# hulop/SfM

Hardware: AMD Instinct MI355X
Metric: BA iterations/sec + residual-evals/sec (cams x pts x obs); 1/2/4/8 GPU (higher is better)
Workload: dtype f64; 1 GPU; C3 per GPU: full BA solve (LM + DENSE_SCHUR, Ceres default options); cams=500, points=200000, observations=2000000, points_per_gpu=200000, obs_per_gpu=2000000, views_per_point=10, parallelism=single GPU, reduced_camera_factor=single GPU

## Files before the change

include/sfm_amd.h:

```cpp
#ifndef SFM_AMD_H_
#define SFM_AMD_H_

#include <stdint.h>

#ifdef __cplusplus
extern "C" {
#endif

#define SFM_ABI_VERSION 1

#define SFM_OK 0
#define SFM_EINVAL (-22)
#define SFM_ENOMEM (-12)
#define SFM_ENODEV (-19)
#define SFM_EIO (-5)
#define SFM_ENOTSUP (-95)

#define SFM_BA_STRUCT_ONLY 0
#define SFM_BA_POSE_ONLY 1
#define SFM_BA_STRUCT_AND_POSE 2

typedef struct sfm_ba_options {
  int32_t max_num_iterations;
  int32_t max_num_consecutive_invalid_steps;
// ... 36 lines not shown
  int32_t step_is_valid;
  int32_t step_is_successful;
  int32_t reserved;
  double cost;
  double cost_change;
  double gradient_max_norm;
  double step_norm;
  double relative_decrease;
  double trust_region_radius;
} sfm_ba_iteration;

typedef struct sfm_ba_handle sfm_ba_handle;

int32_t sfm_abi_version(void);
const char* sfm_last_error(void);
void sfm_ba_default_options(sfm_ba_options* opts);
int32_t sfm_device_count(void);

int sfm_ba_solve(const sfm_ba_options* opts, int32_t mode, int64_t n_obs, const double* obs_uv,
                 const int32_t* cam_idx, const int32_t* pt_idx, int32_t n_cams, const double* K9, double* rot,
                 double* t, int32_t n_pts, double* X, sfm_ba_summary* summary, sfm_ba_iteration* trace,
                 int32_t trace_cap, int32_t* trace_len);

int sfm_ba_create(int32_t device, sfm_ba_handle** out);
int sfm_ba_destroy(sfm_ba_handle* h);
int sfm_ba_set_problem(sfm_ba_handle* h, int64_t n_obs, const double* obs_uv, const int32_t* cam_idx,
                       const int32_t* pt_idx, int32_t n_cams, const double* K9, const double* rot, const double* t,
                       int32_t n_pts, const double* X);
int sfm_ba_reset_parameters(sfm_ba_handle* h);
int sfm_ba_solve_resident(sfm_ba_handle* h, const sfm_ba_options* opts, int32_t mode, sfm_ba_summary* summary,
                          sfm_ba_iteration* trace, int32_t trace_cap, int32_t* trace_len);
int sfm_ba_get_parameters(sfm_ba_handle* h, double* rot, double* t, double* X);
int sfm_ba_evaluate(sfm_ba_handle* h, double* cost, double* res, double* jac);
int sfm_ba_bench_jacobian(sfm_ba_handle* h, int32_t reps, double* avg_ms);
int sfm_ba_phase_times(sfm_ba_handle* h, double* ms9);
int sfm_ba_set_profiling(sfm_ba_handle* h, int32_t on);
int sfm_ba_sync(sfm_ba_handle* h);

int sfm_comm_unique_id(uint8_t out[128]);
int sfm_ba_set_comm(sfm_ba_handle* h, int32_t nranks, int32_t rank, const uint8_t id[128]);
typedef int (*sfm_allreduce_fn)(double* buf, int64_t count, int32_t op, void* user);
int sfm_ba_set_host_comm(sfm_ba_handle* h, int32_t nranks, int32_t rank, sfm_allreduce_fn fn, void* user);
#define SFM_COLL_ALLREDUCE 0
#define SFM_COLL_BROADCAST 1
#define SFM_COLL_REDUCE_SCATTER 2
#define SFM_COLL_REDUCE 3
typedef int (*sfm_collective_fn)(int32_t kind, double* buf, double* out, int64_t count, int32_t arg, void* user);
int sfm_ba_set_host_collectives(sfm_ba_handle* h, int32_t nranks, int32_t rank, sfm_collective_fn fn, void* user);
int sfm_ba_set_distributed_factor(sfm_ba_handle* h, int32_t panel_tiles);

int sfm_match_features(int32_t device, const double* pts0, const uint8_t* desc0, int32_t n0, const double* pts1,
                       const uint8_t* desc1, int32_t n1, int32_t desc_bytes, double ratio_test, double min_distance,
                       double max_distance, int32_t* idx0, int32_t* idx1, int32_t* n_matches);
int sfm_knn2_hamming(int32_t device, const uint8_t* desc0, int32_t n0, const uint8_t* desc1, int32_t n1,
                     int32_t desc_bytes, int32_t* best_idx, int32_t* best_dist, int32_t* second_idx,
                     int32_t* second_dist);

typedef struct sfm_matcher sfm_matcher;
int sfm_matcher_create(int32_t device, int32_t desc_bytes, sfm_matcher** out);
int sfm_matcher_destroy(sfm_matcher* h);
int sfm_matcher_push_frame(sfm_matcher* h, const double* pts, const double* pts_distorted, const uint8_t* desc,
                           int32_t n);
int sfm_matcher_match_subset(sfm_matcher* h, const int32_t* prev_idx, int32_t n_prev, const int32_t* curr_idx,
                             int32_t n_curr, double ratio_test, double min_distance, double max_distance,
                             int32_t* prev_match, int32_t* curr_match, int32_t* n_matches);
int sfm_matcher_store_keyframe(sfm_matcher* h, int32_t slot, const double* pts, const uint8_t* desc, int32_t n);
// ... 246 lines not shown
```

sfm_amd/_ffi.py:

```python
from __future__ import annotations

import ctypes
import os
from ctypes import POINTER, c_char_p, c_double, c_float, c_int, c_int32, c_int64, c_uint8, c_uint64, c_void_p

import numpy as np

_HERE = os.path.dirname(os.path.abspath(__file__))
LIB_PATH = os.environ.get("SFM_AMD_LIB") or os.path.join(_HERE, "libsfm_amd.so")


class SfmError(RuntimeError):

    def __init__(self, code: int, what: str, msg: str):
        super().__init__(f"{what} failed with {code}: {msg}")
        self.code = code


class BAOptions(ctypes.Structure):
    _fields_ = [
        ("max_num_iterations", c_int32),
        ("max_num_consecutive_invalid_steps", c_int32),
        ("jacobi_scaling", c_int32),
        ("reserved0", c_int32),
# ... 117 lines not shown


class GuidanceResult(ctypes.Structure):
    _fields_ = [
        ("centroid", c_double * 3),
        ("box_center", c_float * 2),
        ("box_size", c_float * 2),
        ("box_angle", c_float),
        ("n_points", c_int32),
        ("n_projected", c_int32),
        ("n_hull", c_int32),
        ("n_accepted", c_int32),
        ("area", c_double),
    ]


_SIGNATURES = {
    "sfm_abi_version": (c_int32, []),
    "sfm_last_error": (c_char_p, []),
    "sfm_ba_default_options": (None, [POINTER(BAOptions)]),
    "sfm_device_count": (c_int32, []),
    "sfm_ba_solve": (c_int, [POINTER(BAOptions), c_int32, c_int64, c_void_p, c_void_p, c_void_p, c_int32, c_void_p,
                             c_void_p, c_void_p, c_int32, c_void_p, POINTER(BASummary), c_void_p, c_int32,
                             POINTER(c_int32)]),
    "sfm_ba_create": (c_int, [c_int32, POINTER(c_void_p)]),
    "sfm_ba_destroy": (c_int, [c_void_p]),
    "sfm_ba_set_problem": (c_int, [c_void_p, c_int64, c_void_p, c_void_p, c_void_p, c_int32, c_void_p, c_void_p,
                                   c_void_p, c_int32, c_void_p]),
    "sfm_ba_reset_parameters": (c_int, [c_void_p]),
    "sfm_ba_solve_resident": (c_int, [c_void_p, POINTER(BAOptions), c_int32, POINTER(BASummary), c_void_p, c_int32,
                                      POINTER(c_int32)]),
    "sfm_ba_get_parameters": (c_int, [c_void_p, c_void_p, c_void_p, c_void_p]),
    "sfm_ba_evaluate": (c_int, [c_void_p, POINTER(c_double), c_void_p, c_void_p]),
    "sfm_ba_bench_jacobian": (c_int, [c_void_p, c_int32, POINTER(c_double)]),
    "sfm_ba_phase_times": (c_int, [c_void_p, c_void_p]),
    "sfm_ba_set_profiling": (c_int, [c_void_p, c_int32]),
    "sfm_ba_sync": (c_int, [c_void_p]),
    "sfm_comm_unique_id": (c_int, [c_void_p]),
    "sfm_ba_set_comm": (c_int, [c_void_p, c_int32, c_int32, c_void_p]),
    "sfm_ba_set_host_comm": (c_int, [c_void_p, c_int32, c_int32, c_void_p, c_void_p]),
    "sfm_ba_set_host_collectives": (c_int, [c_void_p, c_int32, c_int32, c_void_p, c_void_p]),
    "sfm_ba_set_distributed_factor": (c_int, [c_void_p, c_int32]),
    "sfm_match_features": (c_int, [c_int32, c_void_p, c_void_p, c_int32, c_void_p, c_void_p, c_int32, c_int32,
                                   c_double, c_double, c_double, c_void_p, c_void_p, POINTER(c_int32)]),
    "sfm_knn2_hamming": (c_int, [c_int32, c_void_p, c_int32, c_void_p, c_int32, c_int32, c_void_p, c_void_p,
                                 c_void_p, c_void_p]),
    "sfm_matcher_create": (c_int, [c_int32, c_int32, POINTER(c_void_p)]),
    "sfm_matcher_destroy": (c_int, [c_void_p]),
    "sfm_matcher_push_frame": (c_int, [c_void_p, c_void_p, c_void_p, c_void_p, c_int32]),
    "sfm_matcher_match_subset": (c_int, [c_void_p, c_void_p, c_int32, c_void_p, c_int32, c_double, c_double, c_double,
                                         c_void_p, c_void_p, POINTER(c_int32)]),
    "sfm_matcher_match_frames": (c_int, [c_void_p, c_int32, c_double, c_double, c_double, c_void_p, c_void_p,
                                         POINTER(c_int32)]),
    "sfm_matcher_match": (c_int, [c_void_p, c_void_p, c_void_p, c_int32, c_void_p, c_void_p, c_int32, c_double,
                                  c_double, c_double, c_void_p, c_void_p, POINTER(c_int32)]),
    "sfm_matcher_knn2": (c_int, [c_void_p, c_void_p, c_int32, c_void_p, c_int32, c_void_p, c_void_p, c_void_p,
                                 c_void_p]),
    "sfm_matcher_last_time": (c_int, [c_void_p, c_void_p]),
    "sfm_representative_descriptors": (c_int, [c_int32, c_void_p, c_void_p, c_int32, c_int32, c_void_p, c_void_p]),
    "sfm_brisk_describe": (c_int, [c_int32, c_void_p, c_int32, c_int32, c_void_p, c_int32, c_void_p, c_void_p,
                                   c_void_p, POINTER(c_int32)]),
    "sfm_klt_brisk_detect_describe": (c_int, [c_void_p, c_int32, c_int32, c_int32, c_void_p, c_void_p, c_void_p,
                                              c_void_p]),
    "sfm_brisk_detect_describe": (c_int, [c_int32, c_void_p, c_int32, c_int32, c_int32, c_int32, c_int32, c_void_p,
                                          c_void_p, c_void_p, POINTER(c_int32)]),
    "sfm_map_create": (c_int, [c_int32, c_int32, POINTER(c_void_p)]),
# ... 197 lines not shown
```

sfm_amd/ba.py:

```python
from __future__ import annotations

import ctypes
from ctypes import c_double, c_int32, c_void_p

import numpy as np

from ._ffi import BAIteration, BAOptions, BASummary, check, default_options, lib, ptr

STRUCT_ONLY, POSE_ONLY, STRUCT_AND_POSE = 0, 1, 2
TERMINATION = {0: "CONVERGENCE", 1: "NO_CONVERGENCE", 2: "FAILURE"}
PHASES = ["jacobian", "cam_reduce", "point_eval", "point_prep", "schur", "cholesky", "backsolve", "backsub", "other"]


def _f64(a) -> np.ndarray:
    return np.ascontiguousarray(a, dtype=np.float64)


def _i32(a) -> np.ndarray:
    return np.ascontiguousarray(a, dtype=np.int32)


def _check_shapes(uv, cam_idx, pt_idx, K9, rot, t, X) -> None:
    n = uv.shape[0] if uv.ndim == 2 else -1
    if uv.ndim != 2 or uv.shape[1] != 2:
# ... 99 lines not shown
        _check_shapes(uv, cam_idx, pt_idx, K9, rot, t, X)
        n = int(uv.shape[0])
        C, P = int(rot.shape[0]), int(X.shape[0])
        check(lib().sfm_ba_set_problem(self._h, n, ptr(uv), ptr(cam_idx), ptr(pt_idx), C, ptr(K9), ptr(rot),
                                       ptr(t), P, ptr(X)), "sfm_ba_set_problem")
        self.n_obs, self.n_cams, self.n_pts = n, C, P

    def reset(self) -> None:
        check(lib().sfm_ba_reset_parameters(self._h), "sfm_ba_reset_parameters")

    def solve(self, options: BAOptions | None = None, mode: int = STRUCT_AND_POSE, trace_cap: int = 128):
        opts = options if options is not None else default_options()
        sm = BASummary()
        tr = (BAIteration * trace_cap)()
        tl = c_int32(0)
        check(lib().sfm_ba_solve_resident(self._h, ctypes.byref(opts), mode, ctypes.byref(sm), tr, trace_cap,
                                          ctypes.byref(tl)), "sfm_ba_solve_resident")
        return sm, [tr[i].as_dict() for i in range(tl.value)]

    def parameters(self):
        rot = np.zeros((self.n_cams, 3))
        t = np.zeros((self.n_cams, 3))
        X = np.zeros((self.n_pts, 3))
        check(lib().sfm_ba_get_parameters(self._h, ptr(rot), ptr(t), ptr(X)), "sfm_ba_get_parameters")
        return rot, t, X

    def evaluate(self, want_jacobian: bool = True):
        cost = c_double(0.0)
        res = np.zeros((self.n_obs, 2))
        jac = np.zeros((self.n_obs, 2, 9)) if want_jacobian else None
        check(lib().sfm_ba_evaluate(self._h, ctypes.byref(cost), ptr(res), ptr(jac)), "sfm_ba_evaluate")
        return cost.value, res, jac

    def bench_jacobian(self, reps: int) -> float:
        ms = c_double(0.0)
        check(lib().sfm_ba_bench_jacobian(self._h, reps, ctypes.byref(ms)), "sfm_ba_bench_jacobian")
        return ms.value

    def set_profiling(self, on: bool) -> None:
        check(lib().sfm_ba_set_profiling(self._h, 1 if on else 0), "sfm_ba_set_profiling")

    def phase_times(self) -> dict:
        buf = np.zeros(2 * len(PHASES))
        check(lib().sfm_ba_phase_times(self._h, ptr(buf)), "sfm_ba_phase_times")
        return {p: {"ms": float(buf[i]), "count": int(buf[len(PHASES) + i])} for i, p in enumerate(PHASES)}

    def sync(self) -> None:
        check(lib().sfm_ba_sync(self._h), "sfm_ba_sync")


def solve(uv, cam_idx, pt_idx, K9, rot, t, X, options: BAOptions | None = None, mode: int = STRUCT_AND_POSE,
          trace_cap: int = 128):
    for name, a in (("rot", rot), ("t", t), ("X", X)):
        if not (isinstance(a, np.ndarray) and a.dtype == np.float64 and a.flags["C_CONTIGUOUS"]):
            raise TypeError(f"{name} must be a C-contiguous float64 array (updated in place)")
    uv, K9 = _f64(uv), _f64(K9)
    cam_idx, pt_idx = _i32(cam_idx), _i32(pt_idx)
    _check_shapes(uv, cam_idx, pt_idx, K9, rot, t, X)
    opts = options if options is not None else default_options()
    sm = BASummary()
    tr = (BAIteration * trace_cap)()
    tl = c_int32(0)
    check(lib().sfm_ba_solve(ctypes.byref(opts), mode, int(uv.shape[0]), ptr(uv), ptr(cam_idx), ptr(pt_idx),
                             int(rot.shape[0]), ptr(K9), ptr(rot), ptr(t), int(X.shape[0]), ptr(X),
                             ctypes.byref(sm), tr, trace_cap, ctypes.byref(tl)), "sfm_ba_solve")
    return sm, [tr[i].as_dict() for i in range(tl.value)]
# ... 24 lines not shown
```

sfm_amd/csrc/ba_kernels.hip:

```cpp
#include <hip/hip_runtime.h>
#include <cfloat>
#include <cmath>
#include <cstdlib>
#include <type_traits>
#include "ba_device.h"
#include "ba_common.h"

namespace sfm {

namespace {

__global__ __launch_bounds__(kThreads) void k_cam_prep(int C, double* __restrict__ cam,
                                                       double* __restrict__ camR, double* __restrict__ part_xn, const int* __restrict__ gate,
                                                       const double* __restrict__ cam_src, const double* __restrict__ X_src,
                                                       double* __restrict__ X_dst, int64_t n_x) {
  if (gate && *gate == 0) return;
  __shared__ double sh[4];
  const int c = blockIdx.x * blockDim.x + threadIdx.x;
  for (int64_t i = int64_t(blockIdx.x) * blockDim.x + threadIdx.x; i < n_x; i += int64_t(gridDim.x) * blockDim.x)
    X_dst[i] = X_src[i];
  if (int64_t(blockIdx.x) * blockDim.x >= C) return;
  double xn = 0.0;
  if (c < C) {
    const double* cs = cam_src ? cam_src : cam;
// ... 366 lines not shown
#pragma unroll
    for (int j = 0; j < 3; ++j) {
      u[j] = (a0 * cr[j] + a1 * cr[3 + j] + a2 * cr[6 + j]) * sp[j];
      v[j] = (b1 * cr[3 + j] + b2 * cr[6 + j]) * sp[j];
    }
    V[0] += u[0] * u[0] + v[0] * v[0];
    V[1] += u[1] * u[0] + v[1] * v[0]; V[2] += u[1] * u[1] + v[1] * v[1];
    V[3] += u[2] * u[0] + v[2] * v[0]; V[4] += u[2] * u[1] + v[2] * v[1]; V[5] += u[2] * u[2] + v[2] * v[2];
    b[0] += u[0] * r0 + v[0] * r1; b[1] += u[1] * r0 + v[1] * r1; b[2] += u[2] * r0 + v[2] * r1;
  }
  const double cn[3] = {V[0], V[2], V[5]};
  if (mode == 0) {
    for (int k = 0; k < 3; ++k) scale_p[3 * size_t(p) + k] = 1.0 / (1.0 + sqrt(cn[k]));
  } else {
    for (int k = 0; k < 3; ++k) {
      if (!reuse) diag_p[3 * size_t(p) + k] = fmin(fmax(cn[k], min_diag), max_diag);
      g = fmax(g, fabs(b[k] / scale_p[3 * size_t(p) + k]));
      xn += X[3 * size_t(p) + k] * X[3 * size_t(p) + k];
    }
    double* o = ptV + size_t(kPtV) * p;
    st2(o, V[0], V[1]); st2(o + 2, V[2], V[3]); st2(o + 4, V[4], V[5]); st2(o + 6, b[0], b[1]); st2(o + 8, b[2], 0.0);
    if (pf.ptL) {
      double fv[9] = {V[0], V[1], V[2], V[3], V[4], V[5], b[0], b[1], b[2]};
      double fd[3], fx[3] = {Xp[0], Xp[1], Xp[2]}, fs[3] = {sp[0], sp[1], sp[2]};
      for (int k = 0; k < 3; ++k) fd[k] = reuse ? diag_p[3 * size_t(p) + k] : fmin(fmax(cn[k], min_diag), max_diag);
      double radius = pf.radius_dev ? *pf.radius_dev : pf.radius;
      asm volatile("" : "+v"(fv[0]), "+v"(fv[1]), "+v"(fv[2]), "+v"(fv[3]), "+v"(fv[4]), "+v"(fv[5]), "+v"(fv[6]),
                        "+v"(fv[7]), "+v"(fv[8]), "+v"(fd[0]), "+v"(fd[1]), "+v"(fd[2]), "+v"(radius));
      bad = point_factor_body(p, fv, fd, radius, fx, fs, pf.ptL, pf.ptS, pf.ptG);
    }
  }
}

__global__ __launch_bounds__(kThreads) void k_point_eval_rc(int P, const PmStream ps,
                                                            const double* __restrict__ camR,
                                                            const double* __restrict__ cam,
                                                            const double* __restrict__ Kc,
                                                            const double* __restrict__ X,
                                                            double* __restrict__ scale_p, double* __restrict__ diag_p,
                                                            double* __restrict__ ptV, double min_diag, double max_diag,
                                                            int mode, int reuse, double* __restrict__ part_grad,
                                                            double* __restrict__ part_xn, const int* __restrict__ gate,
                                                            const PointFold pf) {
  if (gate && *gate == 0) return;
  __shared__ double sh[4];
  const int p = blockIdx.x * blockDim.x + threadIdx.x;
  double g = 0.0, xn = 0.0, bad = 0.0;
  const CamView cv{camR, cam + 3, Kc, kCamR, 6, 5};
  if (p < P)
    point_eval_body(p, ps, cv, X, scale_p, diag_p, ptV, min_diag, max_diag, mode, reuse, g, xn, pf, bad);
  if (mode == 1) {
    const double rg = block_reduce(g, sh, true);
    if (threadIdx.x == 0) part_grad[blockIdx.x] = rg;
    const double rx = block_reduce(xn, sh, false);
    if (threadIdx.x == 0) part_xn[blockIdx.x] = rx;
    if (pf.ptL) {
      const double rb = block_reduce(bad, sh, true);
      if (threadIdx.x == 0) pf.part_bad[blockIdx.x] = rb;
    }
  }
}

constexpr int kCamE = 17;
template <int kMaxC, int kGroups = 1>
__global__ __launch_bounds__(kThreads * kGroups) void k_point_eval_lds(int P, int C, const PmStream ps,
                                                             const double* __restrict__ camR,
                                                             const double* __restrict__ cam,
                                                             const double* __restrict__ Kc,
                                                             const double* __restrict__ X,
                                                             double* __restrict__ scale_p, double* __restrict__ diag_p,
                                                             double* __restrict__ ptV, double min_diag, double max_diag,
                                                             int mode, int reuse, double* __restrict__ part_grad,
                                                             double* __restrict__ part_xn, const int* __restrict__ gate,
                                                             const CamFold cf, const PointFold pf) {
  if (gate && *gate == 0) return;
  static_assert(kGroups == 1 || kMaxC > 64, "the camera fold runs with one group per workgroup");
  const int nbp = (P + kThreads - 1) / kThreads;
  if (kGroups == 1 && int(blockIdx.x) >= nbp) {
    const int c = (int(blockIdx.x) - nbp) * (kThreads / 64) + int(threadIdx.x >> 6);
    if (c < cf.C) cam_sum_body(c, threadIdx.x & 63, cf);
    return;
  }
  __shared__ double sh[4 * kGroups];
  __shared__ double cst[kMaxC * kCamE];
  for (int i = threadIdx.x; i < C * kCamE; i += blockDim.x) {
    const int c = i / kCamE, j = i - c * kCamE;
    cst[i] = j < 9 ? camR[size_t(kCamR) * c + j] : j < 12 ? cam[6 * size_t(c) + 3 + (j - 9)] : Kc[5 * size_t(c) + (j - 12)];
  }
  __syncthreads();
  const int grp = int(threadIdx.x) / kThreads, tg = int(threadIdx.x) % kThreads;
  const int vb = int(blockIdx.x) * kGroups + grp;
  const int p = vb * kThreads + tg;
  double g = 0.0, xn = 0.0, bad = 0.0;
  const CamView cv{cst, cst + 9, cst + 12, kCamE, kCamE, kCamE};
  if (p < P)
    point_eval_body(p, ps, cv, X, scale_p, diag_p, ptV, min_diag, max_diag, mode, reuse, g, xn, pf, bad);
  if (mode == 1) {
    const int w = int(threadIdx.x) >> 6, l = int(threadIdx.x) & 63;
    __shared__ double shb[4 * kGroups];
    const double wg = wave_max(g), wx = wave_sum(xn);
    if (pf.ptL) {
      const double wb = wave_max(bad);
      if (l == 0) shb[w] = wb;
    }
    if (l == 0) sh[w] = wg;
    __syncthreads();
    double rg = 0.0;
    if (tg == 0) {
      rg = sh[4 * grp];
      for (int i = 1; i < 4; ++i) rg = fmax(rg, sh[4 * grp + i]);
    }
    __syncthreads();
    if (l == 0) sh[w] = wx;
    __syncthreads();
    if (tg == 0 && vb < nbp) {
      double rx = sh[4 * grp];
      for (int i = 1; i < 4; ++i) rx = rx + sh[4 * grp + i];
      part_grad[vb] = rg;
      part_xn[vb] = rx;
      if (pf.ptL) {
        double rb = shb[4 * grp];
        for (int i = 1; i < 4; ++i) rb = fmax(rb, shb[4 * grp + i]);
        pf.part_bad[vb] = rb;
      }
    }
  }
}

__global__ __launch_bounds__(kThreads) void k_point_factor(int P, const double* __restrict__ ptV,
                                                           const double* __restrict__ diag_p, double radius,
// ... 1421 lines not shown
    k_jacobian<false><<<d.plan.jac_blocks, kThreads, 0, s>>>(d.jgrp, d.jchunks, d.cm_p, d.uv_cm, d.Kc, d.cam, d.camR, d.X,
                                                        d.scale_c, d.scale_p, scaled ? 1 : 0, d.jrec, slot(d, kPCost),
                                                        d.jpart, d.gate);
}
void launch_cam_reduce(const DevProblem& d, hipStream_t s) {
  if (d.C) k_cam_sum<<<d.C, 64, 0, s>>>(d.cam_rng, d.jpart, d.Ucam, d.gate);
}
static PmStream pm_stream(const DevProblem& d) {
  return d.plan.wave_major ? PmStream{d.pt_off, d.cam_wm, d.uv_wm, d.woff} : PmStream{d.pt_off, d.cam_pm, d.uv_pm, nullptr};
}
static CamFold cam_fold(const DevProblem& d, int mode, bool count_grad) {
  return CamFold{d.cam_rng, d.jpart, d.Ucam, d.scale_c, d.diag_c, d.min_diag, d.max_diag, mode, d.C,
                 count_grad ? slot(d, kPGradCam) : nullptr};
}
void launch_cam_sum_finalize(const DevProblem& d, int mode, bool count_grad, hipStream_t s) {
  if (d.C) k_cam_sum_finalize<<<d.C, 64, 0, s>>>(cam_fold(d, mode, count_grad), d.gate);
}
void launch_point_eval_with_cams(const DevProblem& d, int mode, bool count_grad, hipStream_t s) {
  const int nb = blocks_for(d.P, kThreads) + (d.C + kThreads / 64 - 1) / (kThreads / 64);
  k_point_eval_lds<64><<<nb, kThreads, 0, s>>>(d.P, d.C, pm_stream(d), d.camR, d.cam, d.Kc, d.X,
                                               d.scale_p, d.diag_p, d.ptV, d.min_diag, d.max_diag, mode, 0,
                                               slot(d, kPGradPt), slot(d, kPXNormPt), d.gate,
                                               cam_fold(d, mode, count_grad), PointFold{});
}
void launch_cam_finalize(const DevProblem& d, int mode, bool reuse_diag, bool count_grad, hipStream_t s) {
  k_cam_finalize<<<blocks_for(d.C, kThreads), kThreads, 0, s>>>(d.C, d.Ucam, d.scale_c, d.diag_c, d.min_diag, d.max_diag, mode,
                                                               reuse_diag ? 1 : 0,
                                                               count_grad ? slot(d, kPGradCam) : nullptr, d.gate);
}
void launch_point_eval(const DevProblem& d, PointPass v, int mode, bool reuse_diag, hipStream_t s, bool factor,
                       double radius) {
  if (d.P == 0) return;
  const int nb = blocks_for(d.P, kThreads);
  const PointFold pf = factor && mode == 1 ? PointFold{radius, d.radius_dev, d.ptL, d.ptS, d.ptG, slot(d, kPBad)}
                                           : PointFold{};
#define SFM_PE_LDS(M_)                                                                                            \
  k_point_eval_lds<M_><<<nb, kThreads, 0, s>>>(d.P, d.C, pm_stream(d), d.camR, d.cam, d.Kc, d.X,      \
                                               d.scale_p, d.diag_p, d.ptV, d.min_diag, d.max_diag, mode,           \
                                               reuse_diag ? 1 : 0, slot(d, kPGradPt), slot(d, kPXNormPt), d.gate,    \
                                               CamFold{}, pf)
  switch (v) {
    case PointPass::Lds64: SFM_PE_LDS(64); break;
    case PointPass::Lds512x2:
      k_point_eval_lds<512, 2><<<blocks_for(d.P, 2 * kThreads), 2 * kThreads, 0, s>>>(
          d.P, d.C, pm_stream(d), d.camR, d.cam, d.Kc, d.X, d.scale_p, d.diag_p, d.ptV, d.min_diag,
          d.max_diag, mode, reuse_diag ? 1 : 0, slot(d, kPGradPt), slot(d, kPXNormPt), d.gate, CamFold{}, pf);
      break;
    case PointPass::Lds512: SFM_PE_LDS(512); break;
    case PointPass::Rc:
      k_point_eval_rc<<<nb, kThreads, 0, s>>>(d.P, pm_stream(d), d.camR, d.cam, d.Kc, d.X, d.scale_p,
                                              d.diag_p, d.ptV, d.min_diag, d.max_diag, mode, reuse_diag ? 1 : 0,
                                              slot(d, kPGradPt), slot(d, kPXNormPt), d.gate, pf);
      break;
  }
#undef SFM_PE_LDS
}
void launch_point_factor(const DevProblem& d, double radius, hipStream_t s) {
  if (d.P) k_point_factor<<<blocks_for(d.P, kThreads), kThreads, 0, s>>>(d.P, d.ptV, d.diag_p, radius, d.ptL,
                                                                         slot(d, kPBad), d.X, d.scale_p, d.ptS, d.gate, d.radius_dev,
                                                                         d.ptG);
}
void launch_point_prep(const DevProblem& d, double radius, hipStream_t s) {
  launch_point_factor(d, radius, s);
  launch_obs_prep(d, s);
}
void launch_jac_obs_prep(const DevProblem& d, hipStream_t s) {
  k_jac_obs_prep<<<d.plan.jac_blocks, kThreads, 0, s>>>(d.jgrp, d.jchunks, d.cm_p, d.uv_cm, d.cam_obs, d.Kc, d.cam, d.camR,
                                                   d.scale_c, d.ptS, slot(d, kPCost), d.jpart, d.dpart, d.gate);
}
void launch_obs_prep(const DevProblem& d, hipStream_t s) {
  if (d.N_pad)
    k_obs_prep_rc<<<obs_xcd_blocks(d), kThreads, 0, s>>>(d.jgrp, d.jchunks, d.cm_p, d.uv_cm, d.cam_obs, d.camR, d.cam,
                                                         d.Kc, d.scale_c, d.ptS, d.dpart, d.gate);
}
void launch_schur(const DevProblem& d, PairPass v, double radius, bool add_diag, hipStream_t s) {
  if (v == PairPass::WgBlocks && d.C) {
    const DiagFold f{d.cam_rng, d.dpart, d.Ucam, d.diag_c, radius, d.radius_dev, add_diag ? 1 : 0, d.C, d.n,
                     (d.n + kNB - 1) / kNB * kNB, d.fail, reinterpret_cast<unsigned long long*>(d.ysol)};
    k_schur_pts<64, kThreads / 64><<<int(d.n_bslots), kThreads, 0, s>>>(d.n_bslots, d.blk, d.seg, d.bpts, d.ptS,
                                                                       d.camR, d.cam, d.Kc, d.scale_c, d.S, d.ld,
                                                                       d.bperm, d.gate, f);
    return;
  }
  launch_schur_diag(d, radius, add_diag, s);
  launch_schur_offdiag(d, v, s);
}
void launch_cam_sum_diag(const DevProblem& d, double radius, bool add_diag, hipStream_t s, bool stage_cams) {
  if (!d.C) return;
// ... 122 lines not shown
```

sfm_amd/csrc/ba_plan.h:

```cpp
#pragma once
#include <algorithm>
#include <cstdint>
#include <cstdlib>

#include "ba_host_layout.h"
#include "../../include/sfm_amd.h"

namespace sfm {

constexpr int kCamPMMax = 512;
constexpr int kAcceptFoldMaxCams = 256;
constexpr int64_t kAcceptFoldMaxX = 3 * 8192;


inline const char* env_get(const char* name) { return std::getenv(name); }
inline bool env_flag(const char* name) {
  const char* v = env_get(name);
  return v && v[0] == '1';
}

struct SolveKnobs {
  bool small_setup = true;
  bool pm_wave_major = true;
  int schur_pts_sub = 0;
  int schur_wg = -1;
  int schur_wgs = 0;
  bool force_pack = false;
  int jac_wg_per_xcd = 0;
  bool eval_split = false;
  bool pe_groups1 = false;
  bool host_lm = false;
  bool lm_unfused = false;
  bool no_accept_fold = false;
  int lm_batch = 0;
};

enum KnobTime { kKnobsProblem = 1, kKnobsSolve = 2 };
using EnvGet = const char* (*)(const char*);

inline void read_knobs(SolveKnobs* k, int when, EnvGet get = env_get) {
  auto not0 = [&](const char* n) { const char* v = get(n); return !(v && v[0] == '0'); };
  auto is1 = [&](const char* n) { const char* v = get(n); return v && v[0] == '1'; };
  if (when & kKnobsProblem) {
    k->small_setup = not0("SFM_SMALL_SETUP");
    k->pm_wave_major = not0("SFM_PM_WAVE_MAJOR");
    k->schur_pts_sub = hostlayout::schur_pts_sub_forced(get("SFM_SCHUR_PTS_SUB"));
    k->schur_wg = hostlayout::schur_wg_forced(get("SFM_SCHUR_WG"));
    const char* v = get("SFM_SCHUR_WGS");
    k->schur_wgs = v ? std::min(1 << 16, std::max(0, std::atoi(v)) + 7) / 8 * 8 : 0;
    k->force_pack = is1("SFM_FORCE_PACK");
    v = get("SFM_JAC_WG_PER_XCD");
    k->jac_wg_per_xcd = v ? std::max(0, std::atoi(v)) : 0;
  }
  if (when & kKnobsSolve) {
    k->eval_split = is1("SFM_EVAL_SPLIT");
    k->pe_groups1 = is1("SFM_PE_GROUPS1");
    k->host_lm = is1("SFM_HOST_LM");
    k->lm_unfused = is1("SFM_LM_UNFUSED");
    k->no_accept_fold = is1("SFM_NO_ACCEPT_FOLD");
    const char* v = get("SFM_LM_BATCH");
    k->lm_batch = v ? std::max(1, std::min(64, std::atoi(v))) : 0;
  }
}


inline int blocks_for(int64_t n, int threads) { return int((n + threads - 1) / threads); }
inline int obs_xcd_blocks(int64_t N_pad, int32_t xcd_slice_max) {
  const int64_t per = xcd_slice_max > 0 ? (int64_t(xcd_slice_max) + 3) / 4 : ((N_pad / 64 + 3) / 4 + 7) / 8;
  return int(8 * std::max<int64_t>(1, per));
}
inline int pt_xcd_blocks(int P) {
  const int64_t per_slice = (int64_t(P) + 7) / 8;
  return int(8 * std::max<int64_t>(1, (per_slice + 255) / 256));
}


struct ProblemShape {
  int C = 0, P = 0;
  int64_t N = 0, N_pad = 0;
  int n_jchunks = 0;
  bool host_counts = false;
  bool small_fits = false;
  int64_t n_pairs = -1;
  int64_t wm_slots = -1;

  int64_t n_blk() const { return int64_t(C) * (C + 1) / 2; }
};

struct ProblemPlan {
  bool small_setup = false;
  bool wave_major = false;
  int schur_pts_sub = 8;
  bool schur_wg_blocks = false;
  bool large_system = false;
// ... 51 lines not shown
enum class PointPass {
  Lds64,
  Lds512x2,
  Lds512,
  Rc,
};
enum class PairPass {
  WgBlocks,
  Pts,
  RotPersistent,
};
enum class Backsub {
  OnePass,
  ThreePass,
};

struct SolveShape {
  int C = 0, P = 0;
  int64_t N_pad = 0;
  int32_t xcd_slice_max = 0;
};

struct SolvePlan {
  int32_t mode = SFM_BA_STRUCT_AND_POSE;
  bool cams_var = true, pts_var = true;
  bool sharded = false;
  LmDriver lm = LmDriver::Host;
  int lm_batch = 0;
  bool prep_folded = false;
  CamSums cam_sums = CamSums::None;
  CamPass cam_pass = CamPass::Jacobian;
  PointPass point_pass = PointPass::Lds64;
  bool stage_cams = false;
  PairPass pair_pass = PairPass::Pts;
  bool cam_records_used = false;
  bool dist_factor = false;
  bool pack_allreduce = false;
  Backsub backsub = Backsub::ThreePass;
  int nb_cost = 1, nb_grad_cam = 1;
  int nb_cam = 1, nb_pt = 1;
  int nb_obs = 1, nb_back = 1;

  bool fused_lm() const { return lm == LmDriver::DeviceFused || lm == LmDriver::DeviceFusedAcceptFold; }
  bool accept_fold() const { return lm == LmDriver::DeviceFusedAcceptFold; }
};

inline SolvePlan plan_solve(const ProblemPlan& pp, const SolveShape& sh, int32_t mode, bool sharded,
                            bool host_callbacks, int dist_pt, const SolveKnobs& k) {
  SolvePlan s;
  const int C = sh.C, P = sh.P;
  const bool both = mode == SFM_BA_STRUCT_AND_POSE;
  s.mode = mode;
  s.cams_var = mode != SFM_BA_STRUCT_ONLY;
  s.pts_var = mode != SFM_BA_POSE_ONLY;
  s.sharded = sharded;
  s.dist_factor = sharded && dist_pt > 0;
  const bool host_lm = host_callbacks || s.dist_factor || k.host_lm;
  const bool fuse_lm = !host_lm && !sharded && !k.lm_unfused;
  const bool accept_fold =
      fuse_lm && C > 0 && C <= kAcceptFoldMaxCams && 3 * int64_t(P) <= kAcceptFoldMaxX && !k.no_accept_fold;
  s.lm = host_lm ? LmDriver::Host
                 : accept_fold ? LmDriver::DeviceFusedAcceptFold : fuse_lm ? LmDriver::DeviceFused : LmDriver::Device;
  s.lm_batch = k.lm_batch;
  s.prep_folded = both && !sharded && P > 0 && C > 64 && sh.N_pad > 0 && !pp.schur_wg_blocks;
  s.cam_pass = s.prep_folded && !k.eval_split ? CamPass::JacObsPrep : CamPass::Jacobian;
  const bool cams_in_point_pass = !sharded && s.cams_var && s.pts_var && P > 0 && C > 0 && C <= 64;
  s.cam_sums = cams_in_point_pass ? CamSums::InPointPass
               : s.prep_folded    ? CamSums::SumDiag
               : !s.cams_var      ? CamSums::None
               : sharded          ? CamSums::ReduceAllreduceFinalize
                                  : CamSums::SumFinalize;
  s.point_pass = C <= 64 ? PointPass::Lds64
                 : C <= 512 && !k.pe_groups1 ? PointPass::Lds512x2
                 : C <= 512 ? PointPass::Lds512 : PointPass::Rc;
  s.pair_pass = pp.schur_wg_blocks ? PairPass::WgBlocks : pp.large_system ? PairPass::RotPersistent : PairPass::Pts;
  s.cam_records_used = C > 0 && pp.large_system && pp.xcd_block_order && !pp.schur_wg_blocks;
  s.stage_cams = s.cam_pass == CamPass::JacObsPrep && s.cam_records_used;
  s.pack_allreduce = sharded || pp.force_pack;
  s.backsub = pp.pm_backsub && s.cams_var && s.pts_var && P > 0 && sh.N_pad > 0 ? Backsub::OnePass : Backsub::ThreePass;
  s.nb_pt = std::max(1, blocks_for(P, 256));
  s.nb_cam = std::max(1, blocks_for(C, 256));
  s.nb_cost = pp.jac_blocks;
  s.nb_grad_cam = s.cams_var && !sharded ? std::max(1, C) : s.nb_cam;
  const bool one = s.backsub == Backsub::OnePass;
  s.nb_obs = one ? s.nb_pt : sh.N_pad ? obs_xcd_blocks(sh.N_pad, sh.xcd_slice_max) : 1;
  s.nb_back = one ? s.nb_pt : P ? pt_xcd_blocks(P) : 1;
  return s;
}

}
```

sfm_amd/csrc/ba_solver.hip:

```cpp
#include <hip/hip_runtime.h>
#include <rccl/rccl.h>
#include <map>
#include <atomic>

#include <algorithm>
#include <array>
#include <cfloat>
#include <cmath>
#include <cstdio>
#include <cstdlib>
#include <cstring>
#include <limits>
#include <string>
#include <vector>
#include <chrono>

#include "sfm_trace.h"
#include "ba_device.h"
#include "ba_setup.h"
#include "ba_common.h"
#include "ba_host_layout.h"
#include "ba_handle.h"
#include "../../include/sfm_amd.h"

// ... 415 lines not shown
  hipStream_t s = h->stream;
  mark_begin(h, kPhCamRed);
  if (h->plan.sharded) {
    launch_cam_reduce(d, s);
    if (int rc = allreduce(h, d.Ucam, size_t(kUcam) * d.C, ncclSum)) return rc;
    launch_cam_finalize(d, mode, false, mode == 1, s);
  } else {
    launch_cam_sum_finalize(d, mode, mode == 1, s);
  }
  mark_end(h);
  return 0;
}

int evaluate_enqueue(sfm_ba_handle* h, bool first, bool jacobi_scaling) {
  SFM_TRACE("sfm:evaluate");
  DevProblem& d = h->d;
  const SolvePlan& p = h->plan;
  hipStream_t s = h->stream;
  int rc;
  if (h->accept_grid > 0) launch_cam_prep_accept(d, p.cams_var, h->accept_grid, s);
  else if (h->accept_grid == 0) launch_cam_prep(d, d.cam, p.cams_var, s);
  const bool jac_first = p.cam_pass == CamPass::Jacobian;
  const bool cams_alone = p.cam_sums == CamSums::SumFinalize || p.cam_sums == CamSums::ReduceAllreduceFinalize;
  if (first && jacobi_scaling) {
    mark_begin(h, kPhJac);
    launch_jacobian(d, false, s);
    mark_end(h);
    if (p.cam_sums == CamSums::InPointPass) {
      mark_begin(h, kPhPtEval);
      launch_point_eval_with_cams(d, 0, false, s);
      mark_end(h);
    } else {
      if ((cams_alone || p.cam_sums == CamSums::SumDiag) && (rc = cam_sums_enqueue(h, 0))) return rc;
      if (p.pts_var) launch_point_eval(d, p.point_pass, 0, false, s);
    }
  }
  if (jac_first) {
    mark_begin(h, kPhJac);
    launch_jacobian(d, true, s);
    mark_end(h);
  }
  if (cams_alone && (rc = cam_sums_enqueue(h, 1))) return rc;
  if (p.cam_sums == CamSums::None) {
    hipMemsetAsync(d.partials + size_t(kPGradCam) * d.max_blocks, 0, sizeof(double) * p.nb_cam, s);
    hipMemsetAsync(d.partials + size_t(kPXNormCam) * d.max_blocks, 0, sizeof(double) * p.nb_cam, s);
  }
  if (p.cam_sums == CamSums::InPointPass) {
    mark_begin(h, kPhPtEval);
    launch_point_eval_with_cams(d, 1, true, s);
    mark_end(h);
  } else if (p.pts_var) {
    mark_begin(h, kPhPtEval);
    launch_point_eval(d, p.point_pass, 1, false, s, p.prep_folded, h->eval_radius);
    mark_end(h);
    if (p.prep_folded) {
      mark_begin(h, kPhPtPrep);
      if (jac_first) launch_obs_prep(d, s);
      else launch_jac_obs_prep(d, s);
      mark_end(h);
      mark_begin(h, kPhCamRed);
      launch_cam_sum_diag(d, h->eval_radius, h->rank == 0, s, p.stage_cams);
      mark_end(h);
      h->cams_staged = p.stage_cams;
    }
    h->prep_fresh = p.prep_folded;
  } else {
    hipMemsetAsync(d.partials + size_t(kPGradPt) * d.max_blocks, 0, sizeof(double) * p.nb_pt, s);
    hipMemsetAsync(d.partials + size_t(kPXNormPt) * d.max_blocks, 0, sizeof(double) * p.nb_pt, s);
  }
  if (d.N == 0) hipMemsetAsync(d.partials + size_t(kPCost) * d.max_blocks, 0, sizeof(double), s);
  if (d.P == 0) {
    hipMemsetAsync(d.partials + size_t(kPGradPt) * d.max_blocks, 0, sizeof(double), s);
    hipMemsetAsync(d.partials + size_t(kPXNormPt) * d.max_blocks, 0, sizeof(double), s);
  }
  ReduceBatch rb;
  rb.add(kPCost, p.nb_cost, 0, kCost);
  rb.add(kPGradCam, p.nb_grad_cam, 1, kGradMaxCam);
  rb.add(kPGradPt, p.nb_pt, 1, kGradMaxPt);
  rb.add(kPXNormCam, p.nb_cam, 0, kXNorm2Cam);
  rb.add(kPXNormPt, p.nb_pt, 0, kXNorm2Pt);
  reduce_phase(h, rb, false, first ? kTailInit : kTailPost);
  if (p.sharded) {
    if ((rc = allreduce(h, d.scal + kCost, 1, ncclSum))) return rc;
    if ((rc = allreduce(h, d.scal + kGradMaxCam, 2, ncclMax))) return rc;
    if ((rc = allreduce(h, d.scal + kXNorm2Pt, 1, ncclSum))) return rc;
  }
// ... 222 lines not shown
    if (hipHostMalloc(reinterpret_cast<void**>(&h->lm_ctl_host), sizeof(LmCtl)) != hipSuccess) {
      h->lm_ctl_host = nullptr;
      return fail(SFM_ENOMEM, "hipHostMalloc failed (LM control)");
    }
  }
  const int cap = std::max(1, opts.max_num_iterations + 1);
  if (h->lm_trace_cap < cap) {
    if (h->lm_trace) {
      (void)hipStreamSynchronize(s);
      (void)hipHostFree(h->lm_trace);
    }
    h->lm_trace = nullptr;
    h->lm_trace_cap = 0;
    if (hipHostMalloc(reinterpret_cast<void**>(&h->lm_trace), sizeof(sfm_ba_iteration) * size_t(cap)) != hipSuccess) {
      h->lm_trace = nullptr;
      return fail(SFM_ENOMEM, "hipMalloc failed (LM trace)");
    }
    h->lm_trace_cap = cap;
  }
  LmCtl& c = *h->lm_ctl_host;
  c = lm_start(h, opts);
  HIPCHK(hipMemcpyAsync(h->lm_ctl, &c, sizeof(LmCtl), hipMemcpyHostToDevice, s));
  int batch = 3, batch_next = 2;
  if (h->plan.lm_batch) batch = batch_next = h->plan.lm_batch;
  if (opts.max_num_iterations <= 0) batch = 0;
  const bool jac_scaling = opts.jacobi_scaling != 0;
  const int acc_blocks = std::max(1, std::min(1024, blocks_for(6 * int64_t(d.C) + 3 * int64_t(d.P), 256)));
  d.radius_dev = &h->lm_ctl->radius;
  const bool unfused = !h->plan.fused_lm();
  d.gate = nullptr;
  h->eval_radius = c.radius;
  int rc = evaluate_enqueue(h, true, jac_scaling);
  if (rc == 0 && unfused) k_lm_init<<<1, 1, 0, s>>>(h->lm_ctl, d.scal);
  while (rc == 0) {
    for (int b = 0; b < batch && rc == 0; ++b) {
      d.gate = &h->lm_ctl->run_step;
      if ((rc = compute_step_enqueue(h, c.radius))) break;
      d.gate = nullptr;
      if (unfused) k_lm_decide<<<1, 1, 0, s>>>(h->lm_ctl, d.scal, h->lm_trace, h->lm_trace_cap);
      d.gate = &h->lm_ctl->run_eval;
      h->accept_grid = h->plan.accept_fold() ? -1 : acc_blocks;
      rc = evaluate_enqueue(h, false, jac_scaling);
      h->accept_grid = 0;
      if (rc) break;
      d.gate = nullptr;
      if (unfused) k_lm_post<<<1, 1, 0, s>>>(h->lm_ctl, d.scal, h->lm_trace, h->lm_trace_cap);
    }
    if (rc) break;
    timer.mark("batch enqueued");
    if (h->prefetch_params) {
      if (hipMemcpyAsync(h->param_host, d.cam, sizeof(double) * 6 * size_t(d.C), hipMemcpyDeviceToHost, s) != hipSuccess ||
          hipMemcpyAsync(h->param_host + 6 * size_t(d.C), d.X, sizeof(double) * 3 * size_t(d.P), hipMemcpyDeviceToHost,
                         s) != hipSuccess) {
        rc = fail(SFM_EIO, "parameter readback failed");
        break;
      }
    }
    if (hipMemcpyAsync(&c, h->lm_ctl, sizeof(LmCtl), hipMemcpyDeviceToHost, s) != hipSuccess ||
        hipStreamSynchronize(s) != hipSuccess) {
      rc = fail(SFM_EIO, "LM control readback failed");
      break;
    }
    timer.mark("batch synchronised");
    collect_marks(h);
    if (c.done) break;
    if (lm_rearm(h, &c) && hipMemcpyAsync(h->lm_ctl, &c, sizeof(LmCtl), hipMemcpyHostToDevice, s) != hipSuccess) {
      rc = fail(SFM_EIO, "LM control upload failed");
      break;
    }
    batch = batch_next;
  }
  d.gate = nullptr;
  d.radius_dev = nullptr;
  if (rc) return rc;
  rc = lm_report(opts, c, h->lm_trace, h->lm_trace_cap, sm, push, nonfinite);
  if (!rc) h->param_host_valid = h->prefetch_params;
  return rc;
}

// ... 316 lines not shown
  SFM_TRACE("sfm_ba_evaluate");
  if (!h || !h->has_problem) return fail(SFM_EINVAL, "no problem set");
  HIPCHK(hipSetDevice(h->device));
  DevProblem& d = h->d;
  int rc;
  if ((rc = ensure_records(h))) return rc;
  launch_cam_prep(d, d.cam, false, h->stream);
  launch_jacobian(d, false, h->stream, true);
  if (d.N == 0) HIPCHK(hipMemsetAsync(d.partials, 0, sizeof(double), h->stream));
  launch_reduce(d, kPCost, d.plan.jac_blocks_rec, 0, kCost, h->stream);
  std::vector<double> rec(size_t(kJRec) * d.N_pad);
  std::vector<int32_t> order(size_t(d.N)), pos(size_t(d.N));
  if (d.N) {
    HIPCHK(hipMemcpyAsync(rec.data(), d.jrec, sizeof(double) * rec.size(), hipMemcpyDeviceToHost, h->stream));
    HIPCHK(hipMemcpyAsync(order.data(), d.order, sizeof(int32_t) * order.size(), hipMemcpyDeviceToHost, h->stream));
    HIPCHK(hipMemcpyAsync(pos.data(), d.pos, sizeof(int32_t) * pos.size(), hipMemcpyDeviceToHost, h->stream));
  }
  double c = 0;
  HIPCHK(hipMemcpyAsync(&c, d.scal + kCost, sizeof(double), hipMemcpyDeviceToHost, h->stream));
  HIPCHK(hipStreamSynchronize(h->stream));
  if (cost) *cost = c;
  for (int64_t q = 0; q < d.N; ++q) {
    const int64_t i = order[q];
    const double* r = &rec[size_t(kJRec) * pos[q]];
    if (res) { res[2 * i] = r[kRes]; res[2 * i + 1] = r[kRes + 1]; }
    if (jac) {
      double* J = jac + 18 * i;
      for (int row = 0; row < 2; ++row) {
        for (int k = 0; k < 6; ++k) J[9 * row + k] = r[kJC + 6 * row + k];
        for (int k = 0; k < 3; ++k) J[9 * row + 6 + k] = r[kJX + 3 * row + k];
      }
    }
  }
  return 0;
}

int sfm_dist_factor_profile(int32_t device, int32_t n, int32_t nranks, int32_t panel_tiles, double* fac_ms,
                            double* pack_ms, double* unpack_ms, double* upd_ms, double* misc_ms) {
  if (n <= 0 || nranks < 1 || panel_tiles < 1 || !fac_ms || !pack_ms || !unpack_ms || !upd_ms || !misc_ms)
    return fail(SFM_EINVAL, "bad arguments");
  int ndev = 0;
  if (hipGetDeviceCount(&ndev) != hipSuccess || device < 0 || device >= ndev) return fail(SFM_ENODEV, "no device");
  HIPCHK(hipSetDevice(device));
  DevProblem d;
  d.n = n;
  d.ld = ((n + 1 + kNB - 1) / kNB) * kNB;
  d.nblk = d.ld / kNB;
  const int pt = panel_tiles, np = (d.nblk + pt - 1) / pt;
  const size_t bytes = sizeof(double) * size_t(d.ld) * d.ld;
  hipStream_t s = nullptr;
  HIPCHK(hipStreamCreate(&s));
  double *S = nullptr, *invd = nullptr, *ys = nullptr, *buf = nullptr;
  int *fl = nullptr, *flags = nullptr;
  const size_t nflag = d.nblk + 2 * size_t(d.nblk) * d.nblk + 16;
  HIPCHK(hipMalloc(&S, bytes));
  HIPCHK(hipMalloc(&invd, sizeof(double) * size_t(d.nblk) * kNB * kNB));
  HIPCHK(hipMemset(invd, 0, sizeof(double) * size_t(d.nblk) * kNB * kNB));
  HIPCHK(hipMalloc(&flags, sizeof(int) * nflag));
  HIPCHK(hipMemset(flags, 0, sizeof(int) * nflag));
  HIPCHK(hipMalloc(&ys, sizeof(double) * d.ld));
  HIPCHK(hipMalloc(&fl, sizeof(int)));
  HIPCHK(hipMemset(fl, 0, sizeof(int)));
  HIPCHK(hipMalloc(&buf, bytes));
  HIPCHK(hipMemset(buf, 0, bytes));
  d.S = S; d.invL = invd; d.ysol = ys; d.fail = fl; d.flags = flags;
  d.cflags = flags + d.nblk;
// ... 186 lines not shown
```

Baseline: 1.972 billion residual-evals/s (obs x evaluations).

## Fuse point-eval sweeps into one launch and defer trailing batch evaluation

On the first Jacobi-scaled evaluation, a new templated two-sweep mode runs the mode-0 and mode-1 point passes inside a single kernel, replacing two separate launches. This removes one launch and one full re-read of the point streams. The LM loop also holds back the last step's evaluation in each batch until the control readback shows it is needed, so an unneeded evaluation is not enqueued. A probe API is added for checking correctness, and an env knob turns the fused sweep off.

```diff
diff --git a/include/sfm_amd.h b/include/sfm_amd.h
--- a/include/sfm_amd.h
+++ b/include/sfm_amd.h
@@ -92,6 +92,9 @@
                           sfm_ba_iteration* trace, int32_t trace_cap, int32_t* trace_len);
 int sfm_ba_get_parameters(sfm_ba_handle* h, double* rot, double* t, double* X);
 int sfm_ba_evaluate(sfm_ba_handle* h, double* cost, double* res, double* jac);
+int sfm_ba_point_pass_probe(sfm_ba_handle* h, int32_t variant, int32_t two_sweep, double radius, double* scale_p,
+                            double* diag_p, double* ptV, double* ptL, double* ptS, double* ptG, int32_t* has_ptG,
+                            double* part_grad, double* part_xn, double* part_bad);
 int sfm_ba_bench_jacobian(sfm_ba_handle* h, int32_t reps, double* avg_ms);
 int sfm_ba_phase_times(sfm_ba_handle* h, double* ms9);
 int sfm_ba_set_profiling(sfm_ba_handle* h, int32_t on);
diff --git a/sfm_amd/_ffi.py b/sfm_amd/_ffi.py
--- a/sfm_amd/_ffi.py
+++ b/sfm_amd/_ffi.py
@@ -173,6 +173,8 @@
                                       POINTER(c_int32)]),
     "sfm_ba_get_parameters": (c_int, [c_void_p, c_void_p, c_void_p, c_void_p]),
     "sfm_ba_evaluate": (c_int, [c_void_p, POINTER(c_double), c_void_p, c_void_p]),
+    "sfm_ba_point_pass_probe": (c_int, [c_void_p, c_int32, c_int32, c_double] + [c_void_p] * 6 + [POINTER(c_int32)] +
+                                [c_void_p] * 3),
     "sfm_ba_bench_jacobian": (c_int, [c_void_p, c_int32, POINTER(c_double)]),
     "sfm_ba_phase_times": (c_int, [c_void_p, c_void_p]),
     "sfm_ba_set_profiling": (c_int, [c_void_p, c_int32]),
diff --git a/sfm_amd/ba.py b/sfm_amd/ba.py
--- a/sfm_amd/ba.py
+++ b/sfm_amd/ba.py
@@ -155,6 +155,20 @@
         check(lib().sfm_ba_evaluate(self._h, ctypes.byref(cost), ptr(res), ptr(jac)), "sfm_ba_evaluate")
         return cost.value, res, jac
 
+    def point_pass_probe(self, variant: int, two_sweep: bool, radius: float = 1e4) -> dict:
+        P, nb = self.n_pts, (self.n_pts + 255) // 256
+        out = {"scale_p": np.zeros((P, 3)), "diag_p": np.zeros((P, 3)), "ptV": np.zeros((P, 10)),
+               "ptL": np.zeros((P, 10)), "ptS": np.zeros((P, 16)), "ptG": np.zeros((P, 16)),
+               "part_grad": np.zeros(nb), "part_xn": np.zeros(nb), "part_bad": np.zeros(nb)}
+        has = c_int32(0)
+        check(lib().sfm_ba_point_pass_probe(self._h, variant, 1 if two_sweep else 0, radius, ptr(out["scale_p"]),
+                                            ptr(out["diag_p"]), ptr(out["ptV"]), ptr(out["ptL"]), ptr(out["ptS"]),
+                                            ptr(out["ptG"]), ctypes.byref(has), ptr(out["part_grad"]),
+                                            ptr(out["part_xn"]), ptr(out["part_bad"])), "sfm_ba_point_pass_probe")
+        if not has.value:
+            del out["ptG"]
+        return out
+
     def bench_jacobian(self, reps: int) -> float:
         ms = c_double(0.0)
         check(lib().sfm_ba_bench_jacobian(self._h, reps, ctypes.byref(ms)), "sfm_ba_bench_jacobian")
diff --git a/sfm_amd/csrc/ba_kernels.hip b/sfm_amd/csrc/ba_kernels.hip
--- a/sfm_amd/csrc/ba_kernels.hip
+++ b/sfm_amd/csrc/ba_kernels.hip
@@ -422,6 +422,7 @@
   }
 }
 
+template <bool kTwo = false>
 __global__ __launch_bounds__(kThreads) void k_point_eval_rc(int P, const PmStream ps,
                                                             const double* __restrict__ camR,
                                                             const double* __restrict__ cam,
@@ -437,9 +438,15 @@
   const int p = blockIdx.x * blockDim.x + threadIdx.x;
   double g = 0.0, xn = 0.0, bad = 0.0;
   const CamView cv{camR, cam + 3, Kc, kCamR, 6, 5};
-  if (p < P)
-    point_eval_body(p, ps, cv, X, scale_p, diag_p, ptV, min_diag, max_diag, mode, reuse, g, xn, pf, bad);
-  if (mode == 1) {
+  if (p < P) {
+    if (kTwo) {
+      for (int m = mode - 2; m < mode; ++m)
+        point_eval_body(p, ps, cv, X, scale_p, diag_p, ptV, min_diag, max_diag, m, reuse, g, xn, pf, bad);
+    } else {
+      point_eval_body(p, ps, cv, X, scale_p, diag_p, ptV, min_diag, max_diag, mode, reuse, g, xn, pf, bad);
+    }
+  }
+  if (kTwo || mode == 1) {
     const double rg = block_reduce(g, sh, true);
     if (threadIdx.x == 0) part_grad[blockIdx.x] = rg;
     const double rx = block_reduce(xn, sh, false);
@@ -452,7 +459,7 @@
 }
 
 constexpr int kCamE = 17;
-template <int kMaxC, int kGroups = 1>
+template <int kMaxC, int kGroups = 1, bool kTwo = false>
 __global__ __launch_bounds__(kThreads * kGroups) void k_point_eval_lds(int P, int C, const PmStream ps,
                                                              const double* __restrict__ camR,
                                                              const double* __restrict__ cam,
@@ -483,9 +490,15 @@
   const int p = vb * kThreads + tg;
   double g = 0.0, xn = 0.0, bad = 0.0;
   const CamView cv{cst, cst + 9, cst + 12, kCamE, kCamE, kCamE};
-  if (p < P)
-    point_eval_body(p, ps, cv, X, scale_p, diag_p, ptV, min_diag, max_diag, mode, reuse, g, xn, pf, bad);
-  if (mode == 1) {
+  if (p < P) {
+    if (kTwo) {
+      for (int m = mode - 2; m < mode; ++m)
+        point_eval_body(p, ps, cv, X, scale_p, diag_p, ptV, min_diag, max_diag, m, reuse, g, xn, pf, bad);
+    } else {
+      point_eval_body(p, ps, cv, X, scale_p, diag_p, ptV, min_diag, max_diag, mode, reuse, g, xn, pf, bad);
+    }
+  }
+  if (kTwo || mode == 1) {
     const int w = int(threadIdx.x) >> 6, l = int(threadIdx.x) & 63;
     __shared__ double shb[4 * kGroups];
     const double wg = wave_max(g), wx = wave_sum(xn);
@@ -1973,28 +1986,34 @@
                        double radius) {
   if (d.P == 0) return;
   const int nb = blocks_for(d.P, kThreads);
-  const PointFold pf = factor && mode == 1 ? PointFold{radius, d.radius_dev, d.ptL, d.ptS, d.ptG, slot(d, kPBad)}
+  const PointFold pf = factor && mode >= 1 ? PointFold{radius, d.radius_dev, d.ptL, d.ptS, d.ptG, slot(d, kPBad)}
                                            : PointFold{};
-#define SFM_PE_LDS(M_)                                                                                            \
-  k_point_eval_lds<M_><<<nb, kThreads, 0, s>>>(d.P, d.C, pm_stream(d), d.camR, d.cam, d.Kc, d.X,      \
-                                               d.scale_p, d.diag_p, d.ptV, d.min_diag, d.max_diag, mode,           \
-                                               reuse_diag ? 1 : 0, slot(d, kPGradPt), slot(d, kPXNormPt), d.gate,    \
-                                               CamFold{}, pf)
-  switch (v) {
-    case PointPass::Lds64: SFM_PE_LDS(64); break;
-    case PointPass::Lds512x2:
-      k_point_eval_lds<512, 2><<<blocks_for(d.P, 2 * kThreads), 2 * kThreads, 0, s>>>(
-          d.P, d.C, pm_stream(d), d.camR, d.cam, d.Kc, d.X, d.scale_p, d.diag_p, d.ptV, d.min_diag,
-          d.max_diag, mode, reuse_diag ? 1 : 0, slot(d, kPGradPt), slot(d, kPXNormPt), d.gate, CamFold{}, pf);
-      break;
-    case PointPass::Lds512: SFM_PE_LDS(512); break;
-    case PointPass::Rc:
-      k_point_eval_rc<<<nb, kThreads, 0, s>>>(d.P, pm_stream(d), d.camR, d.cam, d.Kc, d.X, d.scale_p,
-                                              d.diag_p, d.ptV, d.min_diag, d.max_diag, mode, reuse_diag ? 1 : 0,
-                                              slot(d, kPGradPt), slot(d, kPXNormPt), d.gate, pf);
-      break;
-  }
+#define SFM_PE_ARGS                                                                                              \
+  d.scale_p, d.diag_p, d.ptV, d.min_diag, d.max_diag, mode, reuse_diag ? 1 : 0, slot(d, kPGradPt),                \
+      slot(d, kPXNormPt), d.gate
+#define SFM_PE_LDS(M_, G_, TWO_)                                                                                 \
+  k_point_eval_lds<M_, G_, TWO_><<<blocks_for(d.P, G_ * kThreads), G_ * kThreads, 0, s>>>(                        \
+      d.P, d.C, pm_stream(d), d.camR, d.cam, d.Kc, d.X, SFM_PE_ARGS, CamFold{}, pf)
+#define SFM_PE_RC(TWO_)                                                                                          \
+  k_point_eval_rc<TWO_><<<nb, kThreads, 0, s>>>(d.P, pm_stream(d), d.camR, d.cam, d.Kc, d.X, SFM_PE_ARGS, pf)
+  if (mode == 2) {
+    switch (v) {
+      case PointPass::Lds64: SFM_PE_LDS(64, 1, true); break;
+      case PointPass::Lds512x2: SFM_PE_LDS(512, 2, true); break;
+      case PointPass::Lds512: SFM_PE_LDS(512, 1, true); break;
+      case PointPass::Rc: SFM_PE_RC(true); break;
+    }
+  } else {
+    switch (v) {
+      case PointPass::Lds64: SFM_PE_LDS(64, 1, false); break;
+      case PointPass::Lds512x2: SFM_PE_LDS(512, 2, false); break;
+      case PointPass::Lds512: SFM_PE_LDS(512, 1, false); break;
+      case PointPass::Rc: SFM_PE_RC(false); break;
+    }
+  }
+#undef SFM_PE_RC
 #undef SFM_PE_LDS
+#undef SFM_PE_ARGS
 }
 void launch_point_factor(const DevProblem& d, double radius, hipStream_t s) {
   if (d.P) k_point_factor<<<blocks_for(d.P, kThreads), kThreads, 0, s>>>(d.P, d.ptV, d.diag_p, radius, d.ptL,
diff --git a/sfm_amd/csrc/ba_plan.h b/sfm_amd/csrc/ba_plan.h
--- a/sfm_amd/csrc/ba_plan.h
+++ b/sfm_amd/csrc/ba_plan.h
@@ -33,6 +33,7 @@
   bool lm_unfused = false;
   bool no_accept_fold = false;
   int lm_batch = 0;
+  bool pe_two_launch = false;
 };
 
 enum KnobTime { kKnobsProblem = 1, kKnobsSolve = 2 };
@@ -60,6 +61,7 @@
     k->no_accept_fold = is1("SFM_NO_ACCEPT_FOLD");
     const char* v = get("SFM_LM_BATCH");
     k->lm_batch = v ? std::max(1, std::min(64, std::atoi(v))) : 0;
+    k->pe_two_launch = is1("SFM_PE_TWO_LAUNCH");
   }
 }
 
@@ -177,6 +179,7 @@
   CamPass cam_pass = CamPass::Jacobian;
   PointPass point_pass = PointPass::Lds64;
   bool stage_cams = false;
+  bool point_two_sweep = false;
   PairPass pair_pass = PairPass::Pts;
   bool cam_records_used = false;
   bool dist_factor = false;
@@ -218,6 +221,8 @@
   s.point_pass = C <= 64 ? PointPass::Lds64
                  : C <= 512 && !k.pe_groups1 ? PointPass::Lds512x2
                  : C <= 512 ? PointPass::Lds512 : PointPass::Rc;
+  s.point_two_sweep = s.pts_var && P > 0 && s.cam_pass == CamPass::JacObsPrep && s.cam_sums == CamSums::SumDiag &&
+                      !k.pe_two_launch;
   s.pair_pass = pp.schur_wg_blocks ? PairPass::WgBlocks : pp.large_system ? PairPass::RotPersistent : PairPass::Pts;
   s.cam_records_used = C > 0 && pp.large_system && pp.xcd_block_order && !pp.schur_wg_blocks;
   s.stage_cams = s.cam_pass == CamPass::JacObsPrep && s.cam_records_used;
diff --git a/sfm_amd/csrc/ba_solver.hip b/sfm_amd/csrc/ba_solver.hip
--- a/sfm_amd/csrc/ba_solver.hip
+++ b/sfm_amd/csrc/ba_solver.hip
@@ -471,7 +471,7 @@
       mark_end(h);
     } else {
       if ((cams_alone || p.cam_sums == CamSums::SumDiag) && (rc = cam_sums_enqueue(h, 0))) return rc;
-      if (p.pts_var) launch_point_eval(d, p.point_pass, 0, false, s);
+      if (p.pts_var && !p.point_two_sweep) launch_point_eval(d, p.point_pass, 0, false, s);
     }
   }
   if (jac_first) {
@@ -490,7 +490,8 @@
     mark_end(h);
   } else if (p.pts_var) {
     mark_begin(h, kPhPtEval);
-    launch_point_eval(d, p.point_pass, 1, false, s, p.prep_folded, h->eval_radius);
+    launch_point_eval(d, p.point_pass, first && jacobi_scaling && p.point_two_sweep ? 2 : 1, false, s, p.prep_folded,
+                      h->eval_radius);
     mark_end(h);
     if (p.prep_folded) {
       mark_begin(h, kPhPtPrep);
@@ -779,19 +780,31 @@
   h->eval_radius = c.radius;
   int rc = evaluate_enqueue(h, true, jac_scaling);
   if (rc == 0 && unfused) k_lm_init<<<1, 1, 0, s>>>(h->lm_ctl, d.scal);
+  auto eval_post = [&]() -> int {
+    d.gate = &h->lm_ctl->run_eval;
+    h->accept_grid = h->plan.accept_fold() ? -1 : acc_blocks;
+    const int e = evaluate_enqueue(h, false, jac_scaling);
+    h->accept_grid = 0;
+    d.gate = nullptr;
+    if (e == 0 && unfused) k_lm_post<<<1, 1, 0, s>>>(h->lm_ctl, d.scal, h->lm_trace, h->lm_trace_cap);
+    return e;
+  };
+  int steps_enqueued = 0;
+  bool eval_held = false;
   while (rc == 0) {
+    if (eval_held && c.run_eval && (rc = eval_post())) break;
+    eval_held = false;
     for (int b = 0; b < batch && rc == 0; ++b) {
       d.gate = &h->lm_ctl->run_step;
       if ((rc = compute_step_enqueue(h, c.radius))) break;
       d.gate = nullptr;
       if (unfused) k_lm_decide<<<1, 1, 0, s>>>(h->lm_ctl, d.scal, h->lm_trace, h->lm_trace_cap);
-      d.gate = &h->lm_ctl->run_eval;
-      h->accept_grid = h->plan.accept_fold() ? -1 : acc_blocks;
-      rc = evaluate_enqueue(h, false, jac_scaling);
-      h->accept_grid = 0;
-      if (rc) break;
-      d.gate = nullptr;
-      if (unfused) k_lm_post<<<1, 1, 0, s>>>(h->lm_ctl, d.scal, h->lm_trace, h->lm_trace_cap);
+      ++steps_enqueued;
+      if (b + 1 == batch && steps_enqueued < opts.max_num_iterations) {
+        eval_held = true;
+        break;
+      }
+      if ((rc = eval_post())) break;
     }
     if (rc) break;
     timer.mark("batch enqueued");
@@ -1174,6 +1187,51 @@
       }
     }
   }
+  return 0;
+}
+
+int sfm_ba_point_pass_probe(sfm_ba_handle* h, int32_t variant, int32_t two_sweep, double radius, double* scale_p,
+                            double* diag_p, double* ptV, double* ptL, double* ptS, double* ptG, int32_t* has_ptG,
+                            double* part_grad, double* part_xn, double* part_bad) {
+  if (!h || !h->has_problem) return fail(SFM_EINVAL, "no problem set");
+  DevProblem& d = h->d;
+  if (variant < 0 || variant > 3 || d.P <= 0 || d.N == 0 || !(radius > 0)) return fail(SFM_EINVAL, "bad arguments");
+  if ((variant == 0 && d.C > 64) || (variant != 3 && d.C > 512))
+    return fail(SFM_EINVAL, "the variant's camera copy does not hold this many cameras");
+  const PointPass v = variant == 0 ? PointPass::Lds64
+                      : variant == 1 ? PointPass::Lds512x2 : variant == 2 ? PointPass::Lds512 : PointPass::Rc;
+  HIPCHK(hipSetDevice(h->device));
+  hipStream_t s = h->stream;
+  sfm_ba_options o;
+  sfm_ba_default_options(&o);
+  d.min_diag = o.min_lm_diagonal;
+  d.max_diag = o.max_lm_diagonal;
+  d.gate = nullptr;
+  d.radius_dev = nullptr;
+  const size_t P = size_t(d.P), nb = size_t(blocks_for(d.P, 256));
+  struct Out { double* host; double* dev; size_t n; };
+  const Out outs[] = {{scale_p, d.scale_p, 3 * P},
+                      {diag_p, d.diag_p, 3 * P},
+                      {ptV, d.ptV, kPtV * P},
+                      {ptL, d.ptL, kPtL * P},
+                      {ptS, d.ptS, kPtS * P},
+                      {ptG, d.ptG, kPtG * P},
+                      {part_grad, d.partials + size_t(kPGradPt) * d.max_blocks, nb},
+                      {part_xn, d.partials + size_t(kPXNormPt) * d.max_blocks, nb},
+                      {part_bad, d.partials + size_t(kPBad) * d.max_blocks, nb}};
+  for (const Out& t : outs)
+    if (t.dev) HIPCHK(hipMemsetAsync(t.dev, 0xFF, sizeof(double) * t.n, s));
+  launch_cam_prep(d, d.cam, true, s);
+  if (two_sweep) {
+    launch_point_eval(d, v, 2, false, s, true, radius);
+  } else {
+    launch_point_eval(d, v, 0, false, s);
+    launch_point_eval(d, v, 1, false, s, true, radius);
+  }
+  for (const Out& t : outs)
+    if (t.dev && t.host) HIPCHK(hipMemcpyAsync(t.host, t.dev, sizeof(double) * t.n, hipMemcpyDeviceToHost, s));
+  HIPCHK(hipStreamSynchronize(s));
+  if (has_ptG) *has_ptG = d.ptG ? 1 : 0;
   return 0;
 }
 
```

After: 1.988 billion residual-evals/s (obs x evaluations) (median of 6 runs). About the same (+0.8%).
